# eikehmueller/IncompressibleEulerHDG

Measured on AMD Instinct MI355X. Metric: million DOF-updates/sec (HDG-IMEX k=2, 1024^2 tri mesh), higher is better.
Workload: dtype f64

## Files before the change

incompressibleeulerhdg_amd/csrc/hdg_engine.hip:

```cpp
#include <hip/hip_runtime.h>

#include <algorithm>
#include <cmath>
#include <complex>
#include <cstdio>
#include <cstdlib>
#include <cstring>
#include <functional>
#include <memory>
#include <string>
#include <vector>

#include "../../include/hdg_mi355x.h"
#include "../../include/hdg_checkpoint.h"
#include "../../include/hdg_transfer.h"
#include "../../include/hdg_tracer_diffusion.h"
#include "../../include/hdg_tracer_walls.h"
#include "../../include/hdg_buoyancy.h"
#include "../../include/hdg_viscosity.h"
#include "../../include/hdg_coriolis.h"
#include "../../include/hdg_drag.h"
#include "../../include/hdg_moving_walls.h"
#include "../../include/hdg_adaptive_dt.h"
#include "../../include/hdg_streamfunction.h"
// ... 534 lines not shown
    if (periodic && c.ny < 4) throw std::string("the periodic mesh needs at least 4 cell rows");
    if (periodic && comm->size > 1 && g.ny < PERIODIC_MIN_ROWS)
      throw std::string("periodic strips need at least ") + std::to_string(PERIODIC_MIN_ROWS) + " cell rows per rank (ny / ranks = " +
          std::to_string(g.ny) + ")";
    if (periodic) {
      g.joff = c.ny + comm->rank * g.ny; g.nyg = 3 * c.ny; g.nyc = g.ny;
      comm->ring = comm->size > 1;
    }
    g.px = periodic ? 1 : 0;
    g.pj0 = periodic ? comm->rank * g.ny : 0;
    g.P = ((c.nx + 1 + 15) / 16) * 16;
    g.G = (long)(g.ny + 2 * GH) * g.P;
    g.R = g.ny + 2 * GH;
    if (opt.row_pad >= 0) g.R += opt.row_pad;
    else {
      for (int pad = 0; pad < 64; pad++) {
        const double t = std::fmod((double)(2L * c.nx * (g.R + pad) * 16L), 524288.0) / 32768.0;
        if ((t >= 2.5 && t <= 7.5) || (t >= 10.5 && t <= 15.5)) { g.R += pad; break; }
      }
    }
    g.Nc = 2L * c.nx * g.R;
    g.elo = g.ehi = 0;
    g.h = Ldom / c.nx;
    g.nbx = (g.nx + bs() - 1) / bs();
    g.nbxc = (g.nx + 1 + bs() - 1) / bs();
    g.rows_xcd = (g.ny + 7) / 8;
    g.rows_xcdc = (g.nyc + 7) / 8;
    g.wskip = 0; g.wgap0 = 0; g.wgapn = 0; g.wrows = g.ny; g.wrowsc = g.nyc;
    g.dbg_nonbr = opt.dbg_nonbr ? 1 : 0;
    g_all = g;
    g_all.nyc = g.ny + (periodic ? 0 : 1);
    g_all.rows_xcdc = (g_all.nyc + 7) / 8;
    g_all.wrowsc = g_all.nyc;
    NQ = 2L * NU * g.Nc; NPv = (long)NP * g.Nc; NLv = 3L * NL * g.G;
    if (NQ * 8L >= (1L << 32))
      throw std::string("mesh too large for one GPU: a velocity vector must stay below 4 GiB (32-bit buffer offsets); "
                        "use more ranks");
    NQb = 2L * NU * 2L * g.nx * g.ny; NPb = (long)NP * 2L * g.nx * g.ny;
    NLb = n_edges() * NL;
    tab = new Tables(K, g.h, c.tau, c.alpha_penalty, c.equispaced_nodes);
    if (periodic) cfg.trace_precond = cfg.trace_precond ? 1 : 0;
    build_dev_tables();
    alloc_state();
    setup_trace_solver();
    HIPCHECK(hipStreamSynchronize(stream));
  }
  ~Engine() {
    if (debug_on() && comm && comm->rank == 0)
      fprintf(stderr, "[comm] halo exchanges: velocity %ld, pressure %ld, trace %ld, vertex rows %ld (%ld of them beside an interior launch); all-reduces %ld; all-gathers %ld; tiled trace preconditioner applications %ld\n",
              n_halo[0], n_halo[1], n_halo[2], n_halo_mg, n_overlapped, n_reduce, n_gather, n_tile_precond);
    if (opt.flow_check && comm && comm->rank == 0)
      fprintf(stderr, "[flow check] %ld skipped exchanges verified, worst relative deviation %.3e\n", fc_count, fc_worst);
    release();
    delete comm;
  }

  void build_dev_tables() {
    const Tables& T = *tab;
    for (int sh = 0; sh < 2; sh++) {
      for (int e = 0; e < 3; e++) {
        dt.N[sh][e] = upload(T.N[sh][e]);
        dt.Nt[sh][e] = upload(transpose(T.N[sh][e], NE, 2 * NU));
        dt.Lift[sh][e] = upload(T.Lift[sh][e]);
        dt.LiftT[sh][e] = upload(transpose(T.Lift[sh][e], 2 * NU, NE));
        dt.Pt[sh][e] = upload(T.Pt[sh][e]);
        dt.ePhi[sh][e] = upload(T.ePhi[sh][e]);
        dt.eGx[sh][e] = upload(T.eGx[sh][e]);
        dt.eGy[sh][e] = upload(T.eGy[sh][e]);
      }
      dt.B[sh] = upload(T.B[sh]); dt.D0[sh] = upload(T.D0[sh]);
      dt.Ainv[sh] = upload(T.Ainv[sh]); dt.W[sh] = upload(T.W[sh]);
      dt.Y[sh] = upload(T.Y[sh]); dt.SK[sh] = upload(T.SK[sh]);
      dt.cPhi[sh] = upload(T.cPhi[sh]); dt.cGx[sh] = upload(T.cGx[sh]); dt.cGy[sh] = upload(T.cGy[sh]);
    }
    dt.cw = upload(T.cw);
    for (int e = 0; e < 3; e++) dt.ew[e] = upload(T.ew[e]);
    for (int t = 0; t < 3; t++)
      for (int v = 0; v < 3; v++) dt.trDinv[t][v] = upload(T.trDinv[t][v]);
    dt.Vu = upload(T.Vu); dt.Vuinv = upload(T.Vuinv); dt.Vp = upload(T.Vp); dt.Vpinv = upload(T.Vpinv);
    dt.Vl = upload(T.Vl); dt.Vlinv = upload(T.Vlinv);
    for (int e = 0; e < 3; e++) { dt.elen[e] = T.elen[e]; dt.enx[e] = T.enx[e]; dt.eny[e] = T.eny[e]; }
    for (int sh = 0; sh < 2; sh++) for (int e = 0; e < 3; e++) dt.sig[sh][e] = T.sig[sh][e];
    dt.h = T.h; dt.tau = T.tau; dt.alpha = T.alpha; dt.nqc = T.nqc; dt.nqe = T.nqe;
  }

  void alloc_state() {
    curQ = dalloc(NQ); curP = dalloc(NPv); curL = dalloc(NLv);
    for (int i = 0; i < s; i++) {
      stQ.push_back(dalloc(NQ)); stP.push_back(dalloc(NPv)); stL.push_back(dalloc(NLv));
      Qtent.push_back(dalloc(NQ));
      if (i < s - 1 || s == 1) Qstar.push_back(dalloc(NQ));
    }
    for (int i = 0; i <= s; i++) { brhs.push_back(dalloc(NQ)); bscale.push_back(1.0); bsep.push_back(0); }
    ch.assign((size_t)s + 1, ChebStage{});
    profile = dalloc(NQ);
    updU = dalloc(NQ); updP = dalloc(NPv); updL = dalloc(NLv); recP = dalloc(NPv); recL = dalloc(NLv);
    wQ1 = dalloc(NQ); wQ2 = dalloc(NQ); wQ3 = dalloc(NQ); wQ4 = dalloc(NQ);
    wP1 = dalloc(NPv); wL1 = dalloc(NLv); wL2 = dalloc(NLv);
    cg_r = dalloc(NLv); cg_z = dalloc(NLv); cg_p = dalloc(NLv); cg_Ap = dalloc(NLv);
    ch_d = dalloc(NLv); ch_r = dalloc(NLv); tr_one = dalloc(NLv);
    ones_c = dalloc(g.Nc);
    cell_ss = dalloc(g.Nc);
    k_fill<<<vec_blocks(g.Nc), 256, 0, stream>>>(g.Nc, ones_c, 1.0);
    d_ones_ptr = upload_ptrs({ones_c});
    int m = std::max(1, cfg.gmres_restart);
    m = std::min(m, MAXV - 1);
    for (int i = 0; i <= m; i++) gm_V.push_back(dalloc(NQ));
    {
      std::vector<const double*> pv(gm_V.begin(), gm_V.end());
      pv.push_back(nullptr);
      pv.push_back(nullptr);
      d_gmV = upload_ptrs(pv);
    }
    void* p = nullptr;
    HIPCHECK(hipMalloc(&p, sizeof(double*) * (std::max(m, MAXV) + 2)));
    allocs.push_back(p);
    d_ptrs = (const double**)p;
    dot_blocks = 8192;
    d_part = dalloc((long)dot_blocks * MAXV);
    d_res = dalloc(MAXV);
    HIPCHECK(hipHostMalloc((void**)&h_res, sizeof(double) * MAXV));
    d_cgs = dalloc(8);
    HIPCHECK(hipHostMalloc((void**)&h_cgs, sizeof(double) * 8));
    HIPCHECK(hipEventCreateWithFlags(&cg_ev, hipEventDisableTiming));
    hQ_dev = dalloc(NQb); hP_dev = dalloc(NPb);
    hL_dev = dalloc(NLb);
    {
      long cap = std::max<long>(GH * 2L * NU * 2L * g.nx, GH * 3L * NL * g.P);
      cap_halo = (size_t)cap;
      hb_slo = dalloc(cap); hb_shi = dalloc(cap); hb_rlo = dalloc(cap); hb_rhi = dalloc(cap);
    }
    for (int i = 0; i < s; i++) { dinv0.push_back(nullptr); dinv1.push_back(nullptr); hybg0.push_back(nullptr); hybg1.push_back(nullptr); dinv_gamma.push_back(-1.0); }
  }

  template <class F> void by_degree(F&& f) const { with_int<1, 2, 3, 4>(K, "degree", f); }
  template <class F> void by_mfma_degree(F&& f) const { with_int<3, 4>(K, "degree of a matrix-core kernel", f); }
  template <class F> void by_pair_degree(F&& f) const { with_int<1, 2>(K, "degree of a pair kernel", f); }
  enum { RHS_W = 0, RHS_P = 1, RHS_BOTH = 2 };
  template <class F> static void by_rhs(const double* rw, const double* rp, F&& f) {
    with_int<RHS_W, RHS_P, RHS_BOTH>((rw && !rp) ? RHS_W : ((!rw && rp) ? RHS_P : RHS_BOTH), "right-hand sides", f);
  }

  bool halo_on = true;
  long n_halo[3] = {0, 0, 0}, n_reduce = 0, n_gather = 0;
  long n_halo_mg = 0;
  long n_tile_precond = 0;
  enum { LC_ADV = 0, LC_LIFT, LC_RHS, LC_WDIV, LC_CONDENSE, LC_TRACE_APPLY, LC_TRACE_SMOOTH, LC_BACKSUB, LC_MG, LC_VEC, LC_DOT,
         LC_COPY, LC_OTHER, LC_N };
  long lc_calls[HDG_N_LAUNCH_CLASSES] = {0};
  double lc_bytes[HDG_N_LAUNCH_CLASSES] = {0};
  static_assert(LC_N == HDG_N_LAUNCH_CLASSES, "launch classes out of step with the header");
  void tally(int c, double bytes) { lc_calls[c]++; lc_bytes[c] += bytes; }
  double bQ() const { return 8.0 * (double)NQb; }
  double bP() const { return 8.0 * (double)NPb; }
  double bL() const { return 8.0 * (double)NLb; }
  double bvec(long n) const {
    if (n == NQ) return bQ();
    if (n == NPv) return bP();
    if (n == NLv) return bL();
    if (n == g.Nc) return 8.0 * 2.0 * g.nx * g.ny;
    return 8.0 * (double)n;
  }
  bool has_lo() const { return periodic || (comm->size > 1 && comm->rank > 0); }
  bool has_hi() const { return periodic || (comm->size > 1 && comm->rank < comm->size - 1); }
  void halo_rows(double* v, long plane_stride, int row_len, int nplanes, int kind, int depth = 1, int gh = GH) {
    if (periodic && comm->size == 1 && halo_on) {
// ... 128 lines not shown
  Geo window_boundary(const Geo& full) const {
    Geo c = full;
    const int lo = has_lo() ? 1 : 0, hi = has_hi() ? 1 : 0;
    c.wskip = 0;
    c.wgap0 = full.elo + lo;
    c.wgapn = full.ny - lo - hi;
    c.wrows = full.elo + lo + hi + full.ehi;
    c.wrowsc = c.wrows;
    c.rows_xcd = (c.wrows + 7) / 8;
    c.rows_xcdc = (c.wrowsc + 7) / 8;
    return c;
  }
  static Geo corner_gap(Geo c, const Geo& full, int lo, int hi) { c.wgapn = full.nyc - lo - hi; return c; }
  hipStream_t cstream = nullptr;
  hipEvent_t ev_in = nullptr, ev_halo = nullptr;
  bool overlap_on = false;
  long n_overlapped = 0;
  void halo_run(const Pending& pd) {
    if (!pd.on) return;
    if (!cstream) {
      HIPCHECK(hipStreamCreateWithFlags(&cstream, hipStreamNonBlocking));
      HIPCHECK(hipEventCreateWithFlags(&ev_in, hipEventDisableTiming));
      HIPCHECK(hipEventCreateWithFlags(&ev_halo, hipEventDisableTiming));
    }
    HIPCHECK(hipStreamWaitEvent(cstream, ev_in, 0));
    hipStream_t saved = stream;
    stream = cstream;
    try {
      if (pd.kind == FQ) halo_Q(pd.v, pd.depth); else halo_L(pd.v, pd.depth);
    } catch (...) { stream = saved; throw; }
    stream = saved;
    HIPCHECK(hipEventRecord(ev_halo, cstream));
    HIPCHECK(hipStreamWaitEvent(stream, ev_halo, 0));
    n_overlapped++;
  }
  void halo_mark(const Pending& pd) {
    if (!pd.on) return;
    if (!cstream) {
      HIPCHECK(hipStreamCreateWithFlags(&cstream, hipStreamNonBlocking));
      HIPCHECK(hipEventCreateWithFlags(&ev_in, hipEventDisableTiming));
      HIPCHECK(hipEventCreateWithFlags(&ev_halo, hipEventDisableTiming));
    }
    HIPCHECK(hipEventRecord(ev_in, stream));
  }
  template <class L>
  void stencil_launch(const double* in, int kind, int max_ext, bool corner, const std::vector<const double*>& pw, L&& launch,
                      int* ext_out) {
    Pending pd;
    int ext = std::min(stencil_in(in, kind, &pd), max_ext);
    for (const double* q : pw) ext = pw_in(q, ext);
    const Geo full = g_ext(ext);
    if (ext_out) *ext_out = ext;
    if (pd.on && can_split(full)) {
      const int lo = has_lo() ? 1 : 0, hi = has_hi() ? 1 : 0;
      halo_mark(pd);
      launch(window_interior(full));
      halo_run(pd);
      launch(corner ? corner_gap(window_boundary(full), full, lo, hi) : window_boundary(full));
    } else {
      if (pd.on) { halo_mark(pd); halo_run(pd); }
      launch(full);
    }
  }
  dim3 cell_grid_of(const Geo& c) const { return dim3(8 * c.rows_xcd * 2 * c.nbx, 1, 1); }
  static dim3 corner_grid_of(const Geo& c) { return dim3(8 * c.rows_xcdc * c.nbxc, 1, 1); }

  const double *pgm[2] = {nullptr, nullptr}, *wdm[2] = {nullptr, nullptr}, *wdbm[2] = {nullptr, nullptr};
  bool use_mfma_schur() const {
    return opt.mfma_schur && cfg.degree >= MFMA_MIN_DEGREE && !periodic && !general;
  }
  void ensure_schur_tables(PSet& ps) {
    if (ps.bsm[0]) return;
    for (int sh = 0; sh < 2; sh++) {
      dvec Ai, W_, Y_, SK_;
      tab->poissonBlock(sh, ps.tau, Ai, W_, Y_, SK_);
      ps.bsm[sh] = upload(pack_backsub_mfma(*tab, Ai, W_));
      if (sh == 0) schur_Y0 = Y_; else ps.cdm = upload(pack_condense_mfma(*tab, schur_Y0, Y_));
    }
  }
  dvec schur_Y0;
  dim3 schur_cell_grid() const { return dim3(8 * g.rows_xcd * 2); }
  dim3 schur_corner_grid() const { return dim3(8 * g.rows_xcdc); }
  const double* advm[2] = {nullptr, nullptr};
  const double* liftm_plain[2] = {nullptr, nullptr};
  std::vector<double*> liftm_hyb0, liftm_hyb1;
  bool use_mfma_lift() const {
    return opt.mfma_lift && cfg.degree >= MFMA_MIN_DEGREE && !periodic && !general;
  }
  static constexpr int MFMA_MIN_DEGREE = 3;
  bool use_mfma_adv() const { return opt.mfma_adv && cfg.degree >= MFMA_MIN_DEGREE && !periodic && !general; }
  bool lift_pair() const { return opt.lift_pair && K <= 2 && bs() == 128 && !general; }
  enum class LiftForm { per_thread = 0, pair = 1, mfma = 2, general = 3 };
  enum class AdvForm { per_thread, two_lane, mfma, general };
  LiftForm lift_form() const {
    return general ? LiftForm::general : use_mfma_lift() ? LiftForm::mfma : lift_pair() ? LiftForm::pair : LiftForm::per_thread;
  }
  AdvForm adv_form() const {
    if (general) return AdvForm::general;
    if (use_mfma_adv()) return AdvForm::mfma;
    return (K >= opt.adv_split_lo && K <= opt.adv_split_hi) ? AdvForm::two_lane : AdvForm::per_thread;
  }
  static int form_code(AdvForm f) { return f == AdvForm::general ? 3 : (f == AdvForm::mfma ? 2 : 0); }
  void lift_mfma(const Geo& gx, const double* t0, const double* t1, const double* in, double* out, double* chd_ = nullptr,
                 const double* chx_ = nullptr, double c1 = 0.0, double c2 = 0.0) {
    const dim3 grid(8 * gx.rows_xcd * 2);
    by_mfma_degree([&](auto k) {
      if (chd_) k_edge_lift_mfma<k(), true><<<grid, 64 * HDG_LIFT_MFMA_WAVES, 0, stream>>>(gx, t0, t1, in, out, chd_, chx_, c1, c2);
      else k_edge_lift_mfma<k()><<<grid, 64 * HDG_LIFT_MFMA_WAVES, 0, stream>>>(gx, t0, t1, in, out);
    });
  }
  void g_lift_apply(const double* Gt, const double* x, double* out) {
    tally(LC_LIFT, 2 * bQ() + 8.0 * (double)gm->nc * 2 * NU * 3 * NE);
    by_degree([&](auto k) { k_g_lift<k()><<<(gm->nc + 63) / 64, 64, 0, stream>>>(ggeo, g_nref, Gt, x, out); });
  }
  void bdm(const double* in, double* out) {
    const LiftForm form = lift_form();
    if (form == LiftForm::general) {
      if (g_lift) g_lift_apply(g_lift, in, out);
      else csr(gd.Pi, in, 1.0, 0.0, out);
      return;
    }
    const int ext = stencil_in(in, FQ);
    const Geo gx = g_ext(ext);
    fl.set(out, ext);
    tally(LC_LIFT, 2 * bQ());
    switch (form) {
      case LiftForm::mfma:
        if (!liftm_plain[0])
          for (int sh = 0; sh < 2; sh++) liftm_plain[sh] = upload(pack_lift_mfma(*tab, sh, tab->Lift[sh]));
        lift_mfma(gx, liftm_plain[0], liftm_plain[1], in, out);
        break;
      case LiftForm::pair:
        by_pair_degree([&](auto k) { k_edge_lift_pair<k(), false, 0, false><<<cell_grid_of(gx), 128, 0, stream>>>(gx, dt, in, out, nullptr, nullptr, nullptr, nullptr, nullptr, 0.0, 0.0, nullptr); });
        break;
      default:
        by_degree([&](auto k) { k_edge_lift<k(), false, 0, false><<<cell_grid_of(gx), bs(), 0, stream>>>(gx, dt, in, out, nullptr, nullptr, nullptr, nullptr, nullptr, 0.0, 0.0, nullptr); });
    }
  }
  int lift_ext(const double* in, const double* r, const double* chd_, const double* chx_, double c1) {
    int ext = stencil_in(in, FQ);
    ext = pw_in(r, ext);
    if (chd_) { ext = pw_in(chx_, ext); if (c1 != 0.0) ext = pw_in(chd_, ext); }
    return ext;
  }
  double lift_bytes(bool has_r, bool has_out, bool cheb, double c1) const {
    return bQ() * (1 + (has_r ? 1 : 0) + (has_out ? 1 : 0) + (cheb ? (c1 != 0.0 ? 3 : 2) : 0));
  }
  void bdm_plus_bj(const double* in, double* out, const double* r, const double* D0, const double* D1,
                   double* chd_ = nullptr, double* chx_ = nullptr, double c1 = 0.0, double c2 = 0.0) {
    const int ext = lift_ext(in, r, chd_, chx_, c1);
    const Geo gx = g_ext(ext);
    tally(LC_LIFT, lift_bytes(true, out != nullptr, chd_ != nullptr, c1));
    by_degree([&](auto k) { with_bool(chd_ != nullptr, [&](auto cheb) {
      k_edge_lift<k(), false, 1, cheb()><<<cell_grid_of(gx), bs(), 0, stream>>>(gx, dt, in, out, r, D0, D1, chd_, chx_, c1, c2, nullptr);
    }); });
    fl.set(out, ext); fl.set(chd_, ext);
  }
  void bdm_hybrid(const double* in, double* out, const double* D0, const double* D1, double* chd_ = nullptr,
                  double* chx_ = nullptr, double c1 = 0.0, double c2 = 0.0, double* ss = nullptr) {
    KTimed kt_(*this, chd_ != nullptr ? T_KLIFT : T_KLIFT_PLAIN, fl.active() && (chd_ != nullptr || (out && !ss)));
    tally(LC_LIFT, lift_bytes(false, out != nullptr, chd_ != nullptr, c1));
    std::vector<const double*> pw;
    if (chd_) { pw.push_back(chx_); if (c1 != 0.0) pw.push_back(chd_); }
    int ext = 0;
    const LiftForm form = lift_form();
    stencil_launch(in, FQ, GH, false, pw, [&](const Geo& gx) {
      if (form == LiftForm::mfma && !ss && (out || chd_)) {
        for (size_t q = 0; q < hybg0.size(); q++)
          if (hybg0[q] == D0) { lift_mfma(gx, liftm_hyb0[q], liftm_hyb1[q], in, out, chd_, chx_, c1, c2); return; }
      }
      if (form == LiftForm::pair) {
        by_pair_degree([&](auto k) { with_bool(chd_ != nullptr, [&](auto cheb) {
          k_edge_lift_pair<k(), false, 2, cheb()><<<cell_grid_of(gx), 128, 0, stream>>>(gx, dt, in, out, nullptr, D0, D1, chd_, chx_, c1, c2, ss);
        }); });
        return;
      }
      by_degree([&](auto k) { with_bool(chd_ != nullptr, [&](auto cheb) {
        k_edge_lift<k(), false, 2, cheb()><<<cell_grid_of(gx), bs(), 0, stream>>>(gx, dt, in, out, nullptr, D0, D1, chd_, chx_, c1, c2, ss);
      }); });
    }, &ext);
    fl.set(out, ext); fl.set(chd_, ext);
  }
  void bdm_T(const double* in, double* out) {
    if (general) general_unsupported("the transposed lift (additive preconditioner)");
    const int ext = stencil_in(in, FQ);
    const Geo gx = g_ext(ext);
    tally(LC_LIFT, 2 * bQ());
    by_degree([&](auto k) { k_edge_lift<k(), true, 0, false><<<cell_grid_of(gx), bs(), 0, stream>>>(gx, dt, in, out, nullptr, nullptr, nullptr, nullptr, nullptr, 0.0, 0.0, nullptr); });
    fl.set(out, ext);
  }
  void adv_apply(const double* x, const double* qstar, double* out, double gamma, const double* bsub = nullptr) {
    KTimed kt_(*this, bsub != nullptr ? T_KADV : T_KADV_PLAIN, fl.active());
    const double up = cfg.flux_upwind ? 1.0 : 0.0;
    tally(LC_ADV, bQ() * (bsub ? 4 : 3));
    const AdvForm form = adv_form();
    if (form == AdvForm::general) {
      by_degree([&](auto k) { k_g_adv<k()><<<(ggeo.nc + 63) / 64, 64, 0, stream>>>(ggeo, x, qstar, out, gamma, up, bsub); });
      fl.set(out, 0);
      return;
    }
    if (form == AdvForm::mfma && !advm[0]) {
      if (dt.nqc != (cfg.degree == 3 ? 36 : 64)) throw std::string("cell quadrature size does not match the matrix-core advection kernel");
      if (dt.nqe != (3 * cfg.degree + 5) / 2) throw std::string("edge quadrature size does not match the matrix-core advection kernel");
      for (int sh = 0; sh < 2; sh++) advm[sh] = upload(pack_adv_mfma(*tab, sh));
    }
    int ext = 0;
    stencil_launch(x, FQ, GH, false, {qstar, bsub}, [&](const Geo& g) {
      switch (form) {
        case AdvForm::mfma: {
          const dim3 gridc(8 * g.rows_xcd * 2);
          by_mfma_degree([&](auto k) { with_bool(bsub != nullptr, [&](auto resid) {
            k_adv_mfma<k(), resid()><<<gridc, 512, 0, stream>>>(g, dt, advm[0], advm[1], x, qstar, out, gamma, up, bsub);
          }); });
          break;
        }
        case AdvForm::two_lane: {
          const int cpb = bs() / 2, nbx2 = (g.nx + cpb - 1) / cpb;
          by_degree([&](auto k) { k_adv_apply2<k()><<<dim3(8 * g.rows_xcd * 2 * nbx2), bs(), 0, stream>>>(g, dt, x, qstar, out, gamma, up, bsub); });
          break;
        }
        default:
          by_degree([&](auto k) { with_bool(bsub != nullptr, [&](auto resid) {
            k_adv_apply<k(), resid()><<<cell_grid_of(g), bs(), 0, stream>>>(g, dt, x, qstar, out, gamma, up, bsub);
          }); });
      }
    }, &ext);
    fl.set(out, ext);
  }
  void blockdiag(const double* D0, const double* D1, const double* r, const double* zin, double cz, double* out) {
    tally(LC_LIFT, bQ() * (zin ? 3 : 2));
    by_degree([&](auto k) { k_blockdiag<k()><<<cell_grid(), bs(), 0, stream>>>(g, D0, D1, r, zin, cz, out); });
    fl.set(out, 0);
  }
  void pgrad(const double* a, double ca, const double* b, double cb, const double* p, const double* l, double gamma,
             double* out) {
    if (general) {
      lincomb(NQ, {{a, a ? ca : 0.0}, {b, b ? cb : 0.0}}, out);
      csr(gd.Gp, p, gamma, 1.0, out);
      csr(gd.Gl, l, gamma, 1.0, out);
      return;
    }
    halo_L(l);
    tally(LC_RHS, bQ() * (1 + (a ? 1 : 0) + (b ? 1 : 0)) + bP() + bL());
    if (use_mfma_schur()) {
      if (!pgm[0]) for (int sh = 0; sh < 2; sh++) pgm[sh] = upload(pack_pgrad_mfma(*tab, sh));
      by_mfma_degree([&](auto k) { k_pgrad_mfma<k()><<<schur_cell_grid(), 64 * HDG_SCHUR_WAVES, 0, stream>>>(g, pgm[0], pgm[1], a, ca, b, cb, p, l, gamma, out); });
      return;
    }
    by_degree([&](auto k) { k_pgrad<k()><<<cell_grid(), bs(), 0, stream>>>(g, dt, a, ca, b, cb, p, l, gamma, out); });
  }
  bool glue_kernels() const { return opt.glue_fusion && !general && K <= 2 && !use_mfma_schur(); }
  bool pgrad_terms(const Terms& terms, const double* b, const double* p, const double* l, double gamma, double* out) {
    LinComb lc;
    if (!glue_kernels() || !b || !single_chain(lincomb_terms(terms), lc)) return false;
    halo_L(l);
    tally(LC_RHS, bQ() * (2 + lc.n) + bP() + bL());
    by_degree([&](auto k) {
      if constexpr (k() <= 2) k_pgrad_terms<k()><<<cell_grid(), bs(), 0, stream>>>(g, dt, lc, b, p, l, gamma, out);
    });
    return true;
  }
  void weak_div(const double* q, double sc, double* out, bool broken) {
    if (general) { csr(broken ? gd.Bdiv : gd.Wdiv, q, sc, 0.0, out); return; }
    if (!broken) halo_Q(q);
    tally(LC_WDIV, bQ() + bP());
    if (use_mfma_schur()) {
      const double** tb = broken ? wdbm : wdm;
      if (!tb[0]) for (int sh = 0; sh < 2; sh++) tb[sh] = upload(pack_weakdiv_mfma(*tab, sh, broken));
      by_mfma_degree([&](auto k) { with_bool(broken, [&](auto br) {
        k_weak_div_mfma<k(), br()><<<schur_cell_grid(), 64 * HDG_SCHUR_WAVES, 0, stream>>>(g, tb[0], tb[1], q, sc, out);
      }); });
      return;
    }
    by_degree([&](auto k) { with_bool(broken, [&](auto br) { k_weak_div<k(), br()><<<cell_grid(), bs(), 0, stream>>>(g, dt, q, sc, out); }); });
  }
  void trace_apply(const double* lam, const double* base, double cb, double ct, double* out, int max_ext = GH) {
    if (general) {
      if (base && cb != 0.0) { if (out != base) copy(out, base, NLv); if (cb != 1.0) axpby(NLv, 0.0, out, cb, out); csr(gs().S, lam, ct, 1.0, out); }
      else csr(gs().S, lam, ct, 0.0, out);
      return;
    }
    tally(LC_TRACE_APPLY, bL() * (2 + ((base && cb != 0.0) ? 1 : 0)));
    std::vector<const double*> pw;
    if (cb != 0.0) pw.push_back(base);
    int ext = 0;
    stencil_launch(lam, FL, max_ext, true, pw, [&](const Geo& c) {
      by_degree([&](auto k) { k_trace_apply<k()><<<corner_grid_of(c), bs(), 0, stream>>>(c, pdt(), lam, base, cb, ct, out); });
    }, &ext);
    fl.set(out, ext);
  }
  void trace_smooth(const double* v, const double* base, double cb, double ct, double c1, double c2, double* r_out,
                    double* d_out, double* x, bool xadd, double xv, int mode = 0, double c0 = 0.0, const double* xc = nullptr,
                    const double* xin = nullptr) {
    if (general) general_unsupported("the fused trace smoother (multigrid preconditioner)");
    if (!xin) xin = x;
    if (mode == 2 && x == v) throw std::string("trace_smooth: mode 2 must not write the vector its neighbours read");
    const bool same_base = base == v;
    tally(LC_TRACE_SMOOTH, bL() * (1 + ((base && !same_base) ? 1 : 0) + (r_out ? 1 : 0) + (d_out ? 1 : 0) + (x ? ((xadd && mode != 2 && x != v) ? 2 : 1) : 0))
                               + (mode == 2 ? 8.0 * (g.nx + 1.0) * (g.ny + 1.0) : 0.0));
    std::vector<const double*> pw;
    if (cb != 0.0) pw.push_back(base);
    if (x && xadd && mode != 2) pw.push_back(xin);
    int ext = 0;
    StencilAux aux{0, c0, xc, std::sqrt(dt.elen[0]), std::sqrt(dt.elen[2]), std::sqrt(dt.elen[1])};
    const int xa = mode == 2 ? 2 : (xadd ? 1 : 0);
    stencil_launch(v, FL, mode == 2 ? 2 : GH, true, pw, [&](const Geo& c) {
// ... 4821 lines not shown
```

incompressibleeulerhdg_amd/csrc/hdg_kernels.hpp:

```cpp
#pragma once
#include "hdg_side_rows.hpp"
#include <hip/hip_runtime.h>

namespace hdg {

struct Geo {
  int nx, ny, P;
  int nyg, joff, nyc;
  long G;
  long Nc;
  int R;
  double h;
  int nbx;
  int nbxc;
  int rows_xcd;
  int rows_xcdc;
  int dbg_nonbr;
  int px;
  int pj0;
  int elo, ehi;
  int wskip, wgap0, wgapn, wrows, wrowsc;
};
__device__ __forceinline__ int launch_row(const Geo& g, int r) { return r - g.elo + g.wskip + ((g.wgapn && r >= g.wgap0) ? g.wgapn : 0); }
constexpr int GH = 6;
constexpr int DX_DEFAULT = 4;
__device__ __forceinline__ long rowbase(const Geo& g, int s, int j) { return ((long)s * g.R + (j + GH)) * g.nx; }
__device__ __forceinline__ int xm1(const Geo& g, int i) { return i > 0 ? i - 1 : g.nx - 1; }
__device__ __forceinline__ int xp1(const Geo& g, int i) { return (g.px && i == g.nx - 1) ? 0 : i + 1; }

template <int K>
struct Dim {
  static constexpr int NU = (K + 2) * (K + 3) / 2;
  static constexpr int NP = (K + 1) * (K + 2) / 2;
  static constexpr int NL = K + 1;
  static constexpr int NE = K + 2;
  static constexpr int NX = 2 * NU + NP;
  static constexpr int NT = 3 * NL;
};

struct DevTables {
  const double *N[2][3], *Nt[2][3], *Lift[2][3], *LiftT[2][3], *Pt[2][3];
  const double *B[2], *D0[2], *Ainv[2], *W[2], *Y[2], *SK[2];
  const double *cw, *cPhi[2], *cGx[2], *cGy[2];
  const double *ew[3], *ePhi[2][3], *eGx[2][3], *eGy[2][3];
  const double* trDinv[3][3];
  const double *Vu, *Vuinv, *Vp, *Vpinv, *Vl, *Vlinv;
  double elen[3], enx[3], eny[3], sig[2][3];
  double h, tau, alpha;
  int nqc, nqe;
};

#define HDG_CELL_PROLOGUE                                          \
  const int xcd_ = blockIdx.x & 7, q_ = blockIdx.x >> 3;           \
  const int jj_ = q_ / (2 * g.nbx), rem_ = q_ - jj_ * 2 * g.nbx;   \
  const int s = rem_ / g.nbx;                                      \
  const int i = (rem_ - s * g.nbx) * blockDim.x + threadIdx.x;     \
  const int r_ = xcd_ * g.rows_xcd + jj_;                          \
  const int j = launch_row(g, r_);                                 \
  if (jj_ >= g.rows_xcd || r_ >= g.wrows || i >= g.nx) return;     \
  const long c = rowbase(g, s, j) + i;

__device__ __forceinline__ bool nbr(int s, int e, int i, int j, const Geo& g, long& cn) {
  int in, jn;
  bool ok;
  if (g.dbg_nonbr) { cn = 0; return false; }
  if (s == 0) {
    if (e == 0) { in = i; jn = j - 1; ok = (g.joff + j) > 0; }
    else if (e == 1) { in = i; jn = j; ok = true; }
    else { in = xm1(g, i); jn = j; ok = i > 0 || g.px; }
  } else {
    if (e == 0) { in = i; jn = j + 1; ok = (g.joff + j) < g.nyg - 1; }
    else if (e == 1) { in = i; jn = j; ok = true; }
    else { in = xp1(g, i); jn = j; ok = i < g.nx - 1 || g.px; }
  }
  cn = rowbase(g, 1 - s, jn) + in;
  return ok;
}

__device__ __forceinline__ long edge_off(int s, int e, int i, int j, const Geo& g, int& t) {
  if (e == 0) { t = 0; return (long)(j + s + GH) * g.P + i; }
  if (e == 1) { t = 2; return (long)(j + GH) * g.P + i; }
  t = 1;
  return (long)(j + GH) * g.P + (s ? xp1(g, i) : i);
// ... 441 lines not shown
      D0[r] *= (row < NE) ? (has0 ? 0.5 : 1.0) : 0.5;
      D1[r] *= has2 ? 0.5 : 1.0;
      if (row < 12) dst[w][row][li] = D0[r];
      if (row < 8) dst[w][12 + row][li] = D1[r];
    }
    __builtin_amdgcn_wave_barrier();
    double bd[KD];
#pragma unroll
    for (int kd = 0; kd < KD; kd++) bd[kd] = dst[w][4 * kd + lk][li];
#pragma unroll
    for (int mt = 0; mt < MT; mt++) {
      const hdg_d2 lo = xo[2 * mt], hi = (2 * mt + 1 < KQ) ? xo[(2 * mt + 1 < KQ) ? 2 * mt + 1 : 0] : zero2;
      hdg_v4d Y = {lo.x, lo.y, hi.x, hi.y};
      const int m0 = 8 * mt + lk, m1 = m0 + 4;
      hdg_d2 xa = zero2, xb = zero2, pa = zero2, pb = zero2;
      if (CHEB) {
        xa = ld_pair_lane<NU>(Bx, g.Nc, c, m0); xb = ld_pair_lane<NU>(Bx, g.Nc, c, m1);
        if (c1 != 0.0) { pa = ld_pair_lane<NU>(Bp, g.Nc, c, m0); pb = ld_pair_lane<NU>(Bp, g.Nc, c, m1); }
        else { pa = xa; pb = xb; }
      }
#pragma unroll
      for (int kd = 0; kd < KD; kd++) Y = __builtin_amdgcn_mfma_f64_16x16x4f64(tG[(mt * KD + kd) * 64 + l], bd[kd], Y, 0, 0, 0);
      if (col) {
        if (!CHEB || out) {
          if (m0 < NU) st_pair_lane(Bout, g.Nc, c, m0, hdg_d2{Y[0], Y[1]});
          if (m1 < NU) st_pair_lane(Bout, g.Nc, c, m1, hdg_d2{Y[2], Y[3]});
        }
        if (CHEB) {
          const hdg_d2 na = {fma(c1, xa.x - pa.x, fma(c2, Y[0], xa.x)), fma(c1, xa.y - pa.y, fma(c2, Y[1], xa.y))};
          const hdg_d2 nb = {fma(c1, xb.x - pb.x, fma(c2, Y[2], xb.x)), fma(c1, xb.y - pb.y, fma(c2, Y[3], xb.y))};
          if (m0 < NU) st_pair_lane(Bp, g.Nc, c, m0, na);
          if (m1 < NU) st_pair_lane(Bp, g.Nc, c, m1, nb);
        }
      }
    }
  }
}

#ifndef HDG_ADV_WAVES
#define HDG_ADV_WAVES 1
#endif
template <int K>
__device__ __forceinline__ void adv_facet(const DevTables& T, int s, int e, bool has, double upwind, const double (&x)[2 * Dim<K>::NU],
                                          const double (&qs)[2 * Dim<K>::NU], const double (&xn)[2 * Dim<K>::NU],
                                          double (&F)[2 * Dim<K>::NU]) {
  constexpr int NU = Dim<K>::NU;
  const double* __restrict__ Po = T.ePhi[s][e];
  const double* __restrict__ Pn = T.ePhi[1 - s][e];
  const double nx_ = T.enx[e], ny_ = T.eny[e], sg = T.sig[s][e];
  const double pen = T.alpha / T.elen[e];
  const int nq = T.nqe;
#pragma unroll 1
  for (int q = 0; q < nq; q++) {
    double ox = 0, oy = 0, bx = 0, by = 0, qn = 0;
#pragma unroll
    for (int m = 0; m < NU; m++) {
      const double po = Po[q * NU + m], pn = Pn[q * NU + m];
      ox = fma(po, x[m], ox);
      oy = fma(po, x[NU + m], oy);
      bx = fma(pn, xn[m], bx);
      by = fma(pn, xn[NU + m], by);
      qn = fma(po, fma(nx_, qs[m], ny_ * qs[NU + m]), qn);
    }
    if (!has) bx = by = 0.0;
    const double w = T.ew[e][q];
    const double cf = has ? w * (0.5 * sg * qn - upwind * fabs(qn)) : 0.0;
    const double jx = ox - bx, jy = oy - by;
    const double jn = (jx * nx_ + jy * ny_) * pen * w;
    const double vx = cf * jx - jn * nx_;
    const double vy = cf * jy - jn * ny_;
#pragma unroll
    for (int m = 0; m < NU; m++) {
      const double po = Po[q * NU + m];
      F[m] = fma(po, vx, F[m]);
      F[NU + m] = fma(po, vy, F[NU + m]);
    }
  }
}
#ifndef HDG_ADV_PIPE
#define HDG_ADV_PIPE 1
#endif
template <int K, bool RESID>
__global__ __launch_bounds__(128) __attribute__((amdgpu_waves_per_eu(HDG_ADV_WAVES)))
void k_adv_apply(Geo g, DevTables T, const double* __restrict__ xin,
                                                    const double* __restrict__ qstar, double* __restrict__ out,
                                                    double gamma, double upwind, const double* __restrict__ bsub_) {
  constexpr int NU = Dim<K>::NU, N2 = 2 * NU;
  const double* __restrict__ bsub = RESID ? bsub_ : nullptr;
  HDG_CELL_PROLOGUE
  double x[N2], qs[N2], F[N2];
  load_vel<NU>(xin, g.Nc, c, x);
#if HDG_ADV_NT & 1
  load_vel_nt<NU>(qstar, g.Nc, c, qs);
#else
  load_vel<NU>(qstar, g.Nc, c, qs);
#endif
  long cn0, cn1, cn2;
  const bool has0 = nbr(s, 0, i, j, g, cn0), has1 = nbr(s, 1, i, j, g, cn1), has2 = nbr(s, 2, i, j, g, cn2);
  double xa[N2], xb[N2];
  constexpr bool PIPE = HDG_ADV_PIPE != 0 && K == 2;
  if (PIPE) load_vel<NU>(xin, g.Nc, cn0, xa);
#pragma unroll
  for (int n = 0; n < N2; n++) F[n] = 0.0;
  {
    const double* __restrict__ Phi = T.cPhi[s];
    const double* __restrict__ Gx = T.cGx[s];
    const double* __restrict__ Gy = T.cGy[s];
    const int nq = T.nqc;
#pragma unroll 1
    for (int q = 0; q < nq; q++) {
      double qx = 0, qy = 0, dxx = 0, dxy = 0, dyx = 0, dyy = 0;
#pragma unroll
      for (int m = 0; m < NU; m++) {
        const double ph = Phi[q * NU + m], gx = Gx[q * NU + m], gy = Gy[q * NU + m];
        qx = fma(ph, qs[m], qx);
        qy = fma(ph, qs[NU + m], qy);
        dxx = fma(gx, x[m], dxx);
        dxy = fma(gy, x[m], dxy);
        dyx = fma(gx, x[NU + m], dyx);
        dyy = fma(gy, x[NU + m], dyy);
      }
      const double w = T.cw[q];
      const double ax = -w * (qx * dxx + qy * dxy);
      const double ay = -w * (qx * dyx + qy * dyy);
#pragma unroll
      for (int m = 0; m < NU; m++) {
        const double ph = Phi[q * NU + m];
        F[m] = fma(ph, ax, F[m]);
        F[NU + m] = fma(ph, ay, F[NU + m]);
      }
    }
  }
  if (PIPE) {
    load_vel<NU>(xin, g.Nc, cn1, xb);
    adv_facet<K>(T, s, 0, has0, upwind, x, qs, xa, F);
    load_vel<NU>(xin, g.Nc, cn2, xa);
    adv_facet<K>(T, s, 1, has1, upwind, x, qs, xb, F);
    if (bsub) {
#if HDG_ADV_NT & 2
      load_vel_nt<NU>(bsub, g.Nc, c, xb);
#else
      load_vel<NU>(bsub, g.Nc, c, xb);
#endif
    }
    adv_facet<K>(T, s, 2, has2, upwind, x, qs, xa, F);
  } else {
    load_vel<NU>(xin, g.Nc, cn0, xa);
    adv_facet<K>(T, s, 0, has0, upwind, x, qs, xa, F);
    load_vel<NU>(xin, g.Nc, cn1, xa);
    adv_facet<K>(T, s, 1, has1, upwind, x, qs, xa, F);
    load_vel<NU>(xin, g.Nc, cn2, xa);
    adv_facet<K>(T, s, 2, has2, upwind, x, qs, xa, F);
    if (bsub) {
#if HDG_ADV_NT & 2
      load_vel_nt<NU>(bsub, g.Nc, c, xb);
#else
      load_vel<NU>(bsub, g.Nc, c, xb);
#endif
    }
  }
  if (bsub) {
#pragma unroll
    for (int n = 0; n < N2; n++) F[n] = xb[n] - fma(-gamma, F[n], x[n]);
  } else {
#pragma unroll
    for (int n = 0; n < N2; n++) F[n] = fma(-gamma, F[n], x[n]);
  }
#if HDG_ADV_NT & 4
  store_vel_nt<NU>(out, g.Nc, c, F);
#else
  store_vel<NU>(out, g.Nc, c, F);
#endif
}

__device__ __forceinline__ double pair_swap(double v) { return __shfl_xor(v, 1, 64); }
template <int K>
__global__ __launch_bounds__(128) void k_adv_apply2(Geo g, DevTables T, const double* __restrict__ xin,
                                                     const double* __restrict__ qstar, double* __restrict__ out,
                                                     double gamma, double upwind, const double* __restrict__ bsub) {
  constexpr int NU = Dim<K>::NU;
  const int cpb = blockDim.x >> 1, nbx2 = (g.nx + cpb - 1) / cpb;
  const int xcd_ = blockIdx.x & 7, q_ = blockIdx.x >> 3;
  const int jj_ = q_ / (2 * nbx2), rem_ = q_ - jj_ * 2 * nbx2;
  const int s = rem_ / nbx2;
  const int i = (rem_ - s * nbx2) * cpb + (threadIdx.x >> 1);
  const int a = threadIdx.x & 1;
  const int r_ = xcd_ * g.rows_xcd + jj_;
  const int j = launch_row(g, r_);
  if (jj_ >= g.rows_xcd || r_ >= g.wrows || i >= g.nx) return;
  const long c = rowbase(g, s, j) + i;
  const long cbase = (c << 1) + a;
  const long pstride = g.Nc << 1;
  double x[NU], qs[NU], F[NU];
#pragma unroll
  for (int m = 0; m < NU; m++) { x[m] = xin[cbase + (long)m * pstride]; qs[m] = qstar[cbase + (long)m * pstride]; F[m] = 0.0; }
  {
    const double* __restrict__ Phi = T.cPhi[s];
    const double* __restrict__ Gx = T.cGx[s];
    const double* __restrict__ Gy = T.cGy[s];
    const int nq = T.nqc;
#pragma unroll 1
    for (int q = 0; q < nq; q++) {
      double qa = 0, dx_ = 0, dy_ = 0;
#pragma unroll
      for (int m = 0; m < NU; m++) {
        qa = fma(Phi[q * NU + m], qs[m], qa);
        dx_ = fma(Gx[q * NU + m], x[m], dx_);
        dy_ = fma(Gy[q * NU + m], x[m], dy_);
      }
      const double qb = pair_swap(qa);
      const double qx = a == 0 ? qa : qb, qy = a == 0 ? qb : qa;
      const double av = -T.cw[q] * (qx * dx_ + qy * dy_);
#pragma unroll
      for (int m = 0; m < NU; m++) F[m] = fma(Phi[q * NU + m], av, F[m]);
    }
  }
#pragma unroll
  for (int e = 0; e < 3; e++) {
    long cn;
    const bool has = nbr(s, e, i, j, g, cn);
    double xn[NU];
    if (has) {
#pragma unroll
      for (int m = 0; m < NU; m++) xn[m] = xin[(((long)m * g.Nc + cn) << 1) + a];
    } else {
#pragma unroll
      for (int m = 0; m < NU; m++) xn[m] = 0.0;
    }
    const double* __restrict__ Po = T.ePhi[s][e];
    const double* __restrict__ Pn = T.ePhi[1 - s][e];
    const double na = a == 0 ? T.enx[e] : T.eny[e], sg = T.sig[s][e];
    const double pen = T.alpha / T.elen[e];
    const int nq = T.nqe;
#pragma unroll 1
    for (int q = 0; q < nq; q++) {
// ... 1672 lines not shown
```

incompressibleeulerhdg_amd/csrc/hdg_options.hpp:

```cpp
#pragma once
#include <cstdio>
#include <cstdlib>

namespace hdg {

struct Options {
  bool general_csr_lift = false;
  bool general_block_jacobi = false;
  bool general_gmres = false;
  bool general_coarse = true;
  int amg_max_coarse = 2000;
  bool amg_unfused = false;

  bool overlap = false;
  bool force_rccl = false;
  int row_pad = -1;
  bool dbg_nonbr = false;
  bool flow_check = false;
  bool ext = true;
  bool direct_host = true;

  bool mfma_schur = true;
  bool mfma_condense = false;
  bool mfma_lift = true;
  bool mfma_adv = true;
  bool lift_pair = true;
  int adv_split_lo = 3, adv_split_hi = 3;

  bool gmres_arnoldi = false;
  bool tail_gmres = false;
  int sstep_max = 6;
  double sstep_per_decade = 1.7;
  int cheb_every = 64;
  int cheb_m = 6;
  double cheb_flo = -1.0, cheb_fhi = -1.0;
  double cheb_ell = -1.0;
  int cheb_max_expected = 64;
  int cheb_fine_step = 2;
  double cheb_handover = -1.0;
  int cheb_min_k = 6;
  int cheb_hand_cycle = 8;

  bool trace_fuse = true;
  bool trace_fold = true;
  int trace_smooth_its = 2;
  bool trace_tile = true;
  bool trace_tile_strips = true;
  bool trace_tile_periodic = true;
  int trace_tile3 = -1;
  bool trace_fused_dots = true;
  double trace_cheb_lo = 0.1;
  double trace_backward_tol = 0.0;
  int mg_sweeps = 2;
  int mg_coarse = 2;
  bool mg_fuse = true;
  bool mg_tail = true;
  bool mg_dense_tail = true;
  bool mg_dense_tail_periodic = true;
  bool mg_replicated = false;

  bool cg_host_scalars = false;
  bool cg_two_reductions = false;
  bool cg_split_update = true;
  bool cg_fused_scalars = true;
  int cg_xp_batch = 6;
  double cg_xp_w0 = 1.6;
  double cg_floor_c = 32.0;
  int cg_force_replace = 0;
  bool cg_mass_one_by_one = false;
  bool psi_jacobi = false;

  bool glue_fusion = true;
};

inline Options options_from_env() {
  Options o;
  auto get = [](const char* name) { return std::getenv(name); };
  auto flag = [&](const char* name, bool& f) { if (get(name)) f = true; };
  auto unless = [&](const char* name, bool& f) { if (get(name)) f = false; };
  auto integer = [&](const char* name, int& v) { if (const char* e = get(name)) v = std::atoi(e); };
  auto real = [&](const char* name, double& v) { if (const char* e = get(name)) v = std::atof(e); };
  auto range = [&](const char* name, int& lo, int& hi) { if (const char* e = get(name)) std::sscanf(e, "%d:%d", &lo, &hi); };

  flag("HDG_GENERAL_CSR_LIFT", o.general_csr_lift);
  flag("HDG_GENERAL_BLOCK_JACOBI", o.general_block_jacobi);
  flag("HDG_GENERAL_GMRES", o.general_gmres);
  unless("HDG_GENERAL_NO_COARSE", o.general_coarse);
  integer("HDG_AMG_MAX_COARSE", o.amg_max_coarse);
  flag("HDG_AMG_UNFUSED", o.amg_unfused);

  bool no_overlap = false;
  flag("HDG_OVERLAP", o.overlap);
  flag("HDG_NO_OVERLAP", no_overlap);
  flag("HDG_FORCE_RCCL", o.force_rccl);
  integer("HDG_ROW_PAD", o.row_pad);
  flag("HDG_DBG_NONBR", o.dbg_nonbr);
  flag("HDG_FLOW_CHECK", o.flow_check);
  unless("HDG_NO_EXT", o.ext);
  unless("HDG_NO_DIRECT_HOST", o.direct_host);

  unless("HDG_NO_MFMA_SCHUR", o.mfma_schur);
  flag("HDG_MFMA_CONDENSE", o.mfma_condense);
  unless("HDG_NO_MFMA_LIFT", o.mfma_lift);
  unless("HDG_NO_MFMA_ADV", o.mfma_adv);
  unless("HDG_LIFT_NO_PAIR", o.lift_pair);
  range("HDG_ADV_SPLIT", o.adv_split_lo, o.adv_split_hi);

  flag("HDG_GMRES_ARNOLDI", o.gmres_arnoldi);
  flag("HDG_TAIL_GMRES", o.tail_gmres);
  integer("HDG_SSTEP_MAX", o.sstep_max);
  real("HDG_SSTEP_PER_DECADE", o.sstep_per_decade);
  integer("HDG_CHEB_EVERY", o.cheb_every);
  integer("HDG_CHEB_M", o.cheb_m);
  real("HDG_CHEB_FLO", o.cheb_flo);
  real("HDG_CHEB_FHI", o.cheb_fhi);
  real("HDG_CHEB_ELL", o.cheb_ell);
  integer("HDG_CHEB_MAX_EXPECTED", o.cheb_max_expected);
  integer("HDG_CHEB_FINE_STEP", o.cheb_fine_step);
  real("HDG_CHEB_HANDOVER", o.cheb_handover);
  integer("HDG_CHEB_MIN_K", o.cheb_min_k);
  integer("HDG_CHEB_HAND_CYCLE", o.cheb_hand_cycle);

  unless("HDG_TRACE_NO_FUSE", o.trace_fuse);
  unless("HDG_TRACE_NO_FOLD", o.trace_fold);
  integer("HDG_TRACE_SMOOTH_ITS", o.trace_smooth_its);
  unless("HDG_TRACE_NO_TILE", o.trace_tile);
  unless("HDG_TRACE_NO_TILE_STRIPS", o.trace_tile_strips);
  unless("HDG_TRACE_NO_TILE_PERIODIC", o.trace_tile_periodic);
  integer("HDG_TRACE_TILE3", o.trace_tile3);
  unless("HDG_TRACE_NO_FUSED_DOTS", o.trace_fused_dots);
  real("HDG_TRACE_CHEB_LO", o.trace_cheb_lo);
  real("HDG_TRACE_BACKWARD_TOL", o.trace_backward_tol);
  integer("HDG_MG_SWEEPS", o.mg_sweeps);
  integer("HDG_MG_COARSE", o.mg_coarse);
  unless("HDG_MG_NO_FUSE", o.mg_fuse);
  unless("HDG_MG_NO_TAIL", o.mg_tail);
  unless("HDG_MG_NO_DENSE_TAIL", o.mg_dense_tail);
  flag("HDG_MG_REPLICATED", o.mg_replicated);

  flag("HDG_CG_HOST_SCALARS", o.cg_host_scalars);
  flag("HDG_CG_TWO_REDUCTIONS", o.cg_two_reductions);
  unless("HDG_CG_NO_SPLIT_UPDATE", o.cg_split_update);
  unless("HDG_CG_NO_FUSED_SCALARS", o.cg_fused_scalars);
  integer("HDG_CG_XP_BATCH", o.cg_xp_batch);
  real("HDG_CG_XP_W0", o.cg_xp_w0);
  real("HDG_CG_FLOOR_C", o.cg_floor_c);
  integer("HDG_CG_FORCE_REPLACE", o.cg_force_replace);
  flag("HDG_CG_MASS_ONE_BY_ONE", o.cg_mass_one_by_one);
  flag("HDG_PSI_JACOBI", o.psi_jacobi);

  unless("HDG_NO_GLUE_FUSION", o.glue_fusion);

  o.overlap = o.overlap && !no_overlap;
  o.mg_dense_tail = o.mg_dense_tail && o.mg_tail;
  o.mg_dense_tail_periodic = o.mg_dense_tail && o.mg_fuse;
  o.cg_xp_batch = o.cg_xp_batch < 1 ? 1 : (o.cg_xp_batch > 16 ? 16 : o.cg_xp_batch);
  return o;
}

inline bool debug_on() { static const bool v = std::getenv("HDG_DEBUG") != nullptr; return v; }
inline bool debug_cg() { static const bool v = std::getenv("HDG_DEBUG_CG") != nullptr; return v; }

}
```

Before: 862.4.

## Pack k=2 advection tables into constant-address rows with rotated software prefetch

Adds a packed per-shape table for degree 2 advection. It interleaves gradients, basis values and weights per quadrature point, plus edge headers holding normals, sigma and penalty. A new k_adv_apply reads this table through constant address-space pointers and double-buffers rows: it prefetches the next quadrature row while computing the current one, using sched_barriers and explicit waitcnts. The aim is to hide scalar/table load latency in the per-thread advection kernel that the k=2 path uses. The risk is that the tight scheduling barriers and manual waitcnt could serialize or add register pressure.

New measurement: 872.4, median of 6. No clear change (+1.2%).

```diff
diff --git a/incompressibleeulerhdg_amd/csrc/hdg_adv_rot.hpp b/incompressibleeulerhdg_amd/csrc/hdg_adv_rot.hpp
--- /dev/null
+++ b/incompressibleeulerhdg_amd/csrc/hdg_adv_rot.hpp
@@ -0,0 +1,56 @@
+#pragma once
+#include <string>
+#include <vector>
+
+#include "hdg_tables.hpp"
+
+namespace hdg {
+
+template <int K>
+struct AdvRot {
+  static constexpr int NU = (K + 2) * (K + 3) / 2;
+  static constexpr int NQC = K == 1 ? 7 : 16;
+  static constexpr int NQE = (3 * K + 5) / 2;
+  static constexpr int CROW = 3 * NU + 2;
+  static constexpr int EROW = 2 * NU + 4, ENBR = NU + 2;
+  static constexpr int EHEAD = 8;
+  static constexpr int EBLOCK = EHEAD + NQE * EROW;
+  static constexpr int EDGE0 = (NQC + 1) * CROW;
+  static constexpr int SHAPE = EDGE0 + 3 * EBLOCK;
+  static constexpr int SIZE = 2 * SHAPE + EROW;
+};
+
+template <int K>
+inline std::vector<double> pack_adv_rot(const Tables& T) {
+  using R = AdvRot<K>;
+  constexpr int NU = R::NU;
+  if (T.nu != NU || T.nqc != R::NQC || T.nqe != R::NQE) throw std::string("quadrature sizes do not match the rotated advection kernel");
+  std::vector<double> tab((size_t)R::SIZE, 0.0);
+  for (int s = 0; s < 2; s++) {
+    double* b = tab.data() + (size_t)s * R::SHAPE;
+    for (int q = 0; q < R::NQC; q++) {
+      double* r = b + q * R::CROW;
+      for (int m = 0; m < NU; m++) {
+        r[m] = T.cGx[s][q * NU + m];
+        r[NU + m] = T.cGy[s][q * NU + m];
+        r[2 * NU + m] = T.cPhi[s][q * NU + m];
+      }
+      r[3 * NU] = T.cw[q];
+    }
+    for (int e = 0; e < 3; e++) {
+      double* h = b + R::EDGE0 + e * R::EBLOCK;
+      h[0] = T.enx[e]; h[1] = T.eny[e]; h[2] = T.sig[s][e]; h[3] = T.alpha; h[4] = T.elen[e];
+      for (int q = 0; q < R::NQE; q++) {
+        double* r = h + R::EHEAD + q * R::EROW;
+        for (int m = 0; m < NU; m++) {
+          r[m] = T.ePhi[s][e][q * NU + m];
+          r[R::ENBR + m] = T.ePhi[1 - s][e][q * NU + m];
+        }
+        r[NU] = T.ew[e][q];
+      }
+    }
+  }
+  return tab;
+}
+
+}
diff --git a/incompressibleeulerhdg_amd/csrc/hdg_engine.hip b/incompressibleeulerhdg_amd/csrc/hdg_engine.hip
--- a/incompressibleeulerhdg_amd/csrc/hdg_engine.hip
+++ b/incompressibleeulerhdg_amd/csrc/hdg_engine.hip
@@ -640,6 +640,7 @@
     for (int e = 0; e < 3; e++) { dt.elen[e] = T.elen[e]; dt.enx[e] = T.enx[e]; dt.eny[e] = T.eny[e]; }
     for (int sh = 0; sh < 2; sh++) for (int e = 0; e < 3; e++) dt.sig[sh][e] = T.sig[sh][e];
     dt.h = T.h; dt.tau = T.tau; dt.alpha = T.alpha; dt.nqc = T.nqc; dt.nqe = T.nqe;
+    if (adv_rotated()) adv_rot = upload(pack_adv_rot<2>(T));
   }
 
   void alloc_state() {
@@ -934,6 +935,8 @@
   dim3 schur_cell_grid() const { return dim3(8 * g.rows_xcd * 2); }
   dim3 schur_corner_grid() const { return dim3(8 * g.rows_xcdc); }
   const double* advm[2] = {nullptr, nullptr};
+  const double* adv_rot = nullptr;
+  bool adv_rotated() const { return opt.adv_rotate != 0 && K == 2; }
   const double* liftm_plain[2] = {nullptr, nullptr};
   std::vector<double*> liftm_hyb0, liftm_hyb1;
   bool use_mfma_lift() const {
@@ -1073,7 +1076,13 @@
         }
         default:
           by_degree([&](auto k) { with_bool(bsub != nullptr, [&](auto resid) {
-            k_adv_apply<k(), resid()><<<cell_grid_of(g), bs(), 0, stream>>>(g, dt, x, qstar, out, gamma, up, bsub);
+            if constexpr (k() == 2) {
+              if (adv_rotated()) {
+                k_adv_apply<k(), resid()><<<cell_grid_of(g), bs(), 0, stream>>>(g, adv_rot, x, qstar, out, gamma, up, bsub);
+                return;
+              }
+            }
+            k_adv_apply_unrotated<k(), resid()><<<cell_grid_of(g), bs(), 0, stream>>>(g, dt, x, qstar, out, gamma, up, bsub);
           }); });
       }
     }, &ext);
diff --git a/incompressibleeulerhdg_amd/csrc/hdg_kernels.hpp b/incompressibleeulerhdg_amd/csrc/hdg_kernels.hpp
--- a/incompressibleeulerhdg_amd/csrc/hdg_kernels.hpp
+++ b/incompressibleeulerhdg_amd/csrc/hdg_kernels.hpp
@@ -1,4 +1,5 @@
 #pragma once
+#include "hdg_adv_rot.hpp"
 #include "hdg_side_rows.hpp"
 #include <hip/hip_runtime.h>
 
@@ -606,7 +607,7 @@
 #endif
 template <int K, bool RESID>
 __global__ __launch_bounds__(128) __attribute__((amdgpu_waves_per_eu(HDG_ADV_WAVES)))
-void k_adv_apply(Geo g, DevTables T, const double* __restrict__ xin,
+void k_adv_apply_unrotated(Geo g, DevTables T, const double* __restrict__ xin,
                                                     const double* __restrict__ qstar, double* __restrict__ out,
                                                     double gamma, double upwind, const double* __restrict__ bsub_) {
   constexpr int NU = Dim<K>::NU, N2 = 2 * NU;
@@ -675,6 +676,200 @@
     adv_facet<K>(T, s, 1, has1, upwind, x, qs, xa, F);
     load_vel<NU>(xin, g.Nc, cn2, xa);
     adv_facet<K>(T, s, 2, has2, upwind, x, qs, xa, F);
+    if (bsub) {
+#if HDG_ADV_NT & 2
+      load_vel_nt<NU>(bsub, g.Nc, c, xb);
+#else
+      load_vel<NU>(bsub, g.Nc, c, xb);
+#endif
+    }
+  }
+  if (bsub) {
+#pragma unroll
+    for (int n = 0; n < N2; n++) F[n] = xb[n] - fma(-gamma, F[n], x[n]);
+  } else {
+#pragma unroll
+    for (int n = 0; n < N2; n++) F[n] = fma(-gamma, F[n], x[n]);
+  }
+#if HDG_ADV_NT & 4
+  store_vel_nt<NU>(out, g.Nc, c, F);
+#else
+  store_vel<NU>(out, g.Nc, c, F);
+#endif
+}
+
+typedef const __attribute__((address_space(4))) double* adv_tab_ptr;
+template <int N>
+__device__ __forceinline__ void adv_row(adv_tab_ptr p, double (&r)[N]) {
+#pragma unroll
+  for (int n = 0; n < N; n++) r[n] = p[n];
+}
+__device__ __forceinline__ void adv_fence() { __builtin_amdgcn_sched_barrier(0); }
+__device__ __forceinline__ void adv_pin(double& a, double& b) { asm volatile("" : "+v"(a), "+v"(b)); }
+__device__ __forceinline__ void adv_arrived() {
+  __builtin_amdgcn_sched_barrier(0);
+  __builtin_amdgcn_s_waitcnt(0xC07F);
+  __builtin_amdgcn_sched_barrier(0);
+}
+template <int K>
+__device__ __forceinline__ void adv_facet_trace(const double (&O)[Dim<K>::NU + 1], const double (&N)[Dim<K>::NU], bool has, double upwind,
+                                                double nx_, double ny_, double sg, double pen, const double (&x)[2 * Dim<K>::NU],
+                                                const double (&qs)[2 * Dim<K>::NU], const double (&xn)[2 * Dim<K>::NU], double& vx,
+                                                double& vy) {
+  constexpr int NU = Dim<K>::NU;
+  double ox = 0, oy = 0, bx = 0, by = 0, qn = 0;
+#pragma unroll
+  for (int m = 0; m < NU; m++) {
+    const double po = O[m], pn = N[m];
+    ox = fma(po, x[m], ox);
+    oy = fma(po, x[NU + m], oy);
+    bx = fma(pn, xn[m], bx);
+    by = fma(pn, xn[NU + m], by);
+    qn = fma(po, fma(nx_, qs[m], ny_ * qs[NU + m]), qn);
+  }
+  if (!has) bx = by = 0.0;
+  const double w = O[NU];
+  const double cf = has ? w * fma(0.5 * sg, qn, -(upwind * fabs(qn))) : 0.0;
+  const double jx = ox - bx, jy = oy - by;
+  const double jn = fma(jy, ny_, jx * nx_) * pen * w;
+  vx = fma(cf, jx, -(jn * nx_));
+  vy = fma(cf, jy, -(jn * ny_));
+  adv_pin(vx, vy);
+}
+template <int K>
+__device__ __forceinline__ void adv_facet_test(const double (&O)[Dim<K>::NU + 1], double vx, double vy, double (&F)[2 * Dim<K>::NU]) {
+  constexpr int NU = Dim<K>::NU;
+#pragma unroll
+  for (int m = 0; m < NU; m++) {
+    const double po = O[m];
+    F[m] = fma(po, vx, F[m]);
+    F[NU + m] = fma(po, vy, F[NU + m]);
+  }
+}
+template <int K>
+__device__ __forceinline__ void adv_facet_rot(adv_tab_ptr& ro, bool has, double upwind, const double (&x)[2 * Dim<K>::NU],
+                                              const double (&qs)[2 * Dim<K>::NU], const double (&xn)[2 * Dim<K>::NU],
+                                              double (&F)[2 * Dim<K>::NU]) {
+  using R = AdvRot<K>;
+  constexpr int NU = Dim<K>::NU, ER = R::EROW, NB = R::ENBR;
+  const double nx_ = ro[-8], ny_ = ro[-7], sg = ro[-6];
+  const double pen = ro[-5] / ro[-4];
+  double X[NU + 1], Y[NU], Z[NU + 1], vx, vy;
+  adv_row(ro, X);
+  adv_row(ro + NB, Y);
+#pragma unroll 1
+  for (int q = 0; q + 1 < R::NQE; q += 2, ro += 2 * ER) {
+    adv_arrived();
+    adv_row(ro + ER, Z);
+    adv_fence();
+    adv_facet_trace<K>(X, Y, has, upwind, nx_, ny_, sg, pen, x, qs, xn, vx, vy);
+    adv_arrived();
+    adv_row(ro + ER + NB, Y);
+    adv_fence();
+    adv_facet_test<K>(X, vx, vy, F);
+    adv_arrived();
+    adv_row(ro + 2 * ER, X);
+    adv_fence();
+    adv_facet_trace<K>(Z, Y, has, upwind, nx_, ny_, sg, pen, x, qs, xn, vx, vy);
+    adv_arrived();
+    adv_row(ro + 2 * ER + NB, Y);
+    adv_fence();
+    adv_facet_test<K>(Z, vx, vy, F);
+  }
+  if (R::NQE & 1) {
+    adv_arrived();
+    adv_facet_trace<K>(X, Y, has, upwind, nx_, ny_, sg, pen, x, qs, xn, vx, vy);
+    adv_facet_test<K>(X, vx, vy, F);
+  }
+  ro += (R::NQE & 1) * ER + R::EHEAD;
+  adv_fence();
+}
+template <int K, bool RESID>
+__global__ __launch_bounds__(128) __attribute__((amdgpu_waves_per_eu(HDG_ADV_WAVES)))
+void k_adv_apply(Geo g, const double* __restrict__ tab, const double* __restrict__ xin,
+                                                    const double* __restrict__ qstar, double* __restrict__ out,
+                                                    double gamma, double upwind, const double* __restrict__ bsub_) {
+  using R = AdvRot<K>;
+  constexpr int NU = Dim<K>::NU, N2 = 2 * NU;
+  const double* __restrict__ bsub = RESID ? bsub_ : nullptr;
+  HDG_CELL_PROLOGUE
+  double x[N2], qs[N2], F[N2];
+  load_vel<NU>(xin, g.Nc, c, x);
+#if HDG_ADV_NT & 1
+  load_vel_nt<NU>(qstar, g.Nc, c, qs);
+#else
+  load_vel<NU>(qstar, g.Nc, c, qs);
+#endif
+  long cn0, cn1, cn2;
+  const bool has0 = nbr(s, 0, i, j, g, cn0), has1 = nbr(s, 1, i, j, g, cn1), has2 = nbr(s, 2, i, j, g, cn2);
+  double xa[N2], xb[N2];
+  constexpr bool PIPE = HDG_ADV_PIPE != 0 && K == 2;
+  if (PIPE) load_vel<NU>(xin, g.Nc, cn0, xa);
+#pragma unroll
+  for (int n = 0; n < N2; n++) F[n] = 0.0;
+  adv_tab_ptr row = (adv_tab_ptr)tab + s * R::SHAPE;
+  {
+    double G[2 * NU], P[NU + 1];
+    adv_row(row, G);
+#pragma unroll 1
+    for (int q = 0; q < R::NQC; q++, row += R::CROW) {
+      adv_arrived();
+      adv_row(row + 2 * NU, P);
+      adv_fence();
+      double dxx = 0, dxy = 0, dyx = 0, dyy = 0;
+#pragma unroll
+      for (int m = 0; m < NU; m++) {
+        const double gx = G[m], gy = G[NU + m];
+        dxx = fma(gx, x[m], dxx);
+        dxy = fma(gy, x[m], dxy);
+        dyx = fma(gx, x[NU + m], dyx);
+        dyy = fma(gy, x[NU + m], dyy);
+      }
+      adv_pin(dxx, dxy);
+      adv_pin(dyx, dyy);
+      adv_arrived();
+      adv_row(row + R::CROW, G);
+      adv_fence();
+      double qx = 0, qy = 0;
+#pragma unroll
+      for (int m = 0; m < NU; m++) {
+        const double ph = P[m];
+        qx = fma(ph, qs[m], qx);
+        qy = fma(ph, qs[NU + m], qy);
+      }
+      const double w = P[NU];
+      const double ax = -w * fma(qy, dxy, qx * dxx);
+      const double ay = -w * fma(qy, dyy, qx * dyx);
+#pragma unroll
+      for (int m = 0; m < NU; m++) {
+        const double ph = P[m];
+        F[m] = fma(ph, ax, F[m]);
+        F[NU + m] = fma(ph, ay, F[NU + m]);
+      }
+    }
+    adv_fence();
+  }
+  row += R::CROW + R::EHEAD;
+  if (PIPE) {
+    load_vel<NU>(xin, g.Nc, cn1, xb);
+    adv_facet_rot<K>(row, has0, upwind, x, qs, xa, F);
+    load_vel<NU>(xin, g.Nc, cn2, xa);
+    adv_facet_rot<K>(row, has1, upwind, x, qs, xb, F);
+    if (bsub) {
+#if HDG_ADV_NT & 2
+      load_vel_nt<NU>(bsub, g.Nc, c, xb);
+#else
+      load_vel<NU>(bsub, g.Nc, c, xb);
+#endif
+    }
+    adv_facet_rot<K>(row, has2, upwind, x, qs, xa, F);
+  } else {
+    load_vel<NU>(xin, g.Nc, cn0, xa);
+    adv_facet_rot<K>(row, has0, upwind, x, qs, xa, F);
+    load_vel<NU>(xin, g.Nc, cn1, xa);
+    adv_facet_rot<K>(row, has1, upwind, x, qs, xa, F);
+    load_vel<NU>(xin, g.Nc, cn2, xa);
+    adv_facet_rot<K>(row, has2, upwind, x, qs, xa, F);
     if (bsub) {
 #if HDG_ADV_NT & 2
       load_vel_nt<NU>(bsub, g.Nc, c, xb);
diff --git a/incompressibleeulerhdg_amd/csrc/hdg_options.hpp b/incompressibleeulerhdg_amd/csrc/hdg_options.hpp
--- a/incompressibleeulerhdg_amd/csrc/hdg_options.hpp
+++ b/incompressibleeulerhdg_amd/csrc/hdg_options.hpp
@@ -26,6 +26,7 @@
   bool mfma_adv = true;
   bool lift_pair = true;
   int adv_split_lo = 3, adv_split_hi = 3;
+  int adv_rotate = 1;
 
   bool gmres_arnoldi = false;
   bool tail_gmres = false;
@@ -105,6 +106,7 @@
   unless("HDG_NO_MFMA_ADV", o.mfma_adv);
   unless("HDG_LIFT_NO_PAIR", o.lift_pair);
   range("HDG_ADV_SPLIT", o.adv_split_lo, o.adv_split_hi);
+  integer("HDG_ADV_ROTATE", o.adv_rotate);
 
   flag("HDG_GMRES_ARNOLDI", o.gmres_arnoldi);
   flag("HDG_TAIL_GMRES", o.tail_gmres);
```
